# DaehwanKimLab/centrifuge

Hardware: NVIDIA H100
Metric: reads/sec (100 bp SE classification) (higher is better)
Workload: dtype u64

## Files before the change

centrifuge_b200/csrc/cf_logic.h:

```cpp
#ifndef CF_LOGIC_H_
#define CF_LOGIC_H_

#include <stdint.h>

#ifdef __CUDACC__
#define CFB_HD __host__ __device__ __forceinline__
#define CFB_HDN __host__ __device__
#else
#define CFB_HD inline
#define CFB_HDN inline
#endif

namespace cfb {

static const uint64_t kOff = 0xffffffffffffffffull;
static const uint64_t kUnk = 0xfffffffffffffffeull;
static const uint32_t kBwNone = 0xffffffffu;

struct IndexView {
	const uint64_t* sides;
	const uint64_t* ftab;
	const uint64_t* eftab;
	const uint16_t* sample16;
	const uint32_t* sample32;
// ... 245 lines not shown
	}
};

template <class T, class C> CFB_HD void ss_swap(T& a, T& b, C&) { T t = a; a = b; b = t; }

template <class T, class C> CFB_HDN void ss_unguarded_linear_insert(T* last, C comp) {
	T val = *last; T* next = last - 1;
	while(comp(val, *next)) { *last = *next; last = next; --next; }
	*last = val;
}
template <class T, class C> CFB_HDN void ss_insertion_sort(T* first, T* last, C comp) {
	if(first == last) return;
	for(T* i = first + 1; i != last; ++i) {
		if(comp(*i, *first)) { T val = *i; for(T* q = i; q != first; --q) *q = *(q - 1); *first = val; }
		else ss_unguarded_linear_insert(i, comp);
	}
}
template <class T, class C> CFB_HDN void ss_push_heap(T* first, long hole, long top, T value, C comp) {
	long parent = (hole - 1) / 2;
	while(hole > top && comp(first[parent], value)) { first[hole] = first[parent]; hole = parent; parent = (hole - 1) / 2; }
	first[hole] = value;
}
template <class T, class C> CFB_HDN void ss_adjust_heap(T* first, long hole, long len, T value, C comp) {
	const long top = hole; long child = hole;
	while(child < (len - 1) / 2) {
		child = 2 * (child + 1);
		if(comp(first[child], first[child - 1])) child--;
		first[hole] = first[child]; hole = child;
	}
	if((len & 1) == 0 && child == (len - 2) / 2) { child = 2 * (child + 1); first[hole] = first[child - 1]; hole = child - 1; }
	ss_push_heap(first, hole, top, value, comp);
}
template <class T, class C> CFB_HDN void ss_heapsort(T* first, T* last, C comp) {
	long len = (long)(last - first);
	if(len >= 2) {
		long parent = (len - 2) / 2;
		for(;;) { T v = first[parent]; ss_adjust_heap(first, parent, len, v, comp); if(parent == 0) break; parent--; }
	}
	while(last - first > 1) { --last; T v = *last; *last = *first; ss_adjust_heap(first, 0L, (long)(last - first), v, comp); }
}
template <class T, class C> CFB_HDN T* ss_partition_pivot(T* first, T* last, C comp) {
	T* mid = first + (last - first) / 2;
	T *a = first + 1, *b = mid, *c = last - 1;
	if(comp(*a, *b)) { if(comp(*b, *c)) ss_swap(*first, *b, comp); else if(comp(*a, *c)) ss_swap(*first, *c, comp); else ss_swap(*first, *a, comp); }
	else if(comp(*a, *c)) ss_swap(*first, *a, comp);
	else if(comp(*b, *c)) ss_swap(*first, *c, comp);
	else ss_swap(*first, *b, comp);
	T* lo = first + 1; T* hi = last; T* pivot = first;
	for(;;) {
		while(comp(*lo, *pivot)) ++lo;
		--hi;
		while(comp(*pivot, *hi)) --hi;
		if(!(lo < hi)) return lo;
		ss_swap(*lo, *hi, comp);
		++lo;
	}
}
template <class T, class C> CFB_HDN void std_sort(T* first, T* last, C comp) {
	const long n = (long)(last - first);
	if(n <= 0) return;
	if(n > 16) {
		int lg = 0; for(long t = n; t > 1; t >>= 1) lg++;
		T* st_first[64]; T* st_last[64]; int st_depth[64]; int sp = 0;
		st_first[0] = first; st_last[0] = last; st_depth[0] = 2 * lg; sp = 1;
		while(sp > 0) {
			--sp; T* f = st_first[sp]; T* l = st_last[sp]; int depth = st_depth[sp];
			while(l - f > 16) {
				if(depth == 0) { ss_heapsort(f, l, comp); break; }
				--depth;
				T* cut = ss_partition_pivot(f, l, comp);
				st_first[sp] = cut; st_last[sp] = l; st_depth[sp] = depth; sp++;
				l = cut;
			}
		}
		ss_insertion_sort(first, first + 16, comp);
		for(T* i = first + 16; i != last; ++i) ss_unguarded_linear_insert(i, comp);
	} else ss_insertion_sort(first, last, comp);
}

struct UnitHits {
	HitRec* L[2][2]; uint32_t n[2][2]; uint32_t rdlen[2]; int n_mates;
};

template <class F> CFB_HDN void for_each_visit(const Params& p, const UnitHits& u, F& f) {
	uint64_t maxG = p.khits;
	for(int rdi = 0; rdi < u.n_mates; rdi++) {
		int a, b;
		choose_strand(p, u.L[rdi][0], u.n[rdi][0], u.L[rdi][1], u.n[rdi][1], a, b);
		for(int fwi = a; fwi < b; fwi++) {
			const HitRec* L = u.L[rdi][fwi]; const uint32_t n = u.n[rdi][fwi];
			for(uint32_t hi = 0; hi < n; hi++) if(L[hi].len >= p.min_hitlen && hsize(L[hi]) > maxG) maxG = hsize(L[hi]);
			if(maxG > p.khits) maxG += p.khits;
			f(rdi, fwi, maxG);
		}
	}
}

struct SortAndCount {
	const Params& p; UnitHits& u; uint64_t rows;
	CFB_HD SortAndCount(const Params& p_, UnitHits& u_) : p(p_), u(u_), rows(0) {}
	CFB_HD void operator()(int rdi, int fwi, uint64_t maxG) {
		HitRec* L = u.L[rdi][fwi]; const uint32_t n = u.n[rdi][fwi];
		std_sort(L, L + n, HitLess());
		uint64_t cnt = 0;
		for(uint32_t hi = 0; hi < n; hi++) {
			if(L[hi].len <= p.min_hitlen) continue;
			if(hsize(L[hi]) == 0) continue;
			const uint64_t nelt = hsize(L[hi]) < maxG ? hsize(L[hi]) : maxG;
			if(nelt > p.ihits) continue;
			rows += nelt; cnt += nelt;
			if(cnt >= maxG) break;
		}
	}
};

struct CountRows {
	const Params& p; const UnitHits& u; uint64_t rows;
	CFB_HD CountRows(const Params& p_, const UnitHits& u_) : p(p_), u(u_), rows(0) {}
	CFB_HD void operator()(int rdi, int fwi, uint64_t maxG) {
		const HitRec* L = u.L[rdi][fwi]; const uint32_t n = u.n[rdi][fwi];
		uint64_t cnt = 0;
		for(uint32_t hi = 0; hi < n; hi++) {
			if(L[hi].len <= p.min_hitlen) continue;
			if(hsize(L[hi]) == 0) continue;
			const uint64_t nelt = hsize(L[hi]) < maxG ? hsize(L[hi]) : maxG;
			if(nelt > p.ihits) continue;
			rows += nelt; cnt += nelt;
			if(cnt >= maxG) break;
		}
	}
};

struct EmitRows {
	const Params& p; const UnitHits& u; uint64_t* out; uint64_t k; uint32_t ts, last_ts;
	CFB_HD EmitRows(const Params& p_, const UnitHits& u_, uint64_t* o) : p(p_), u(u_), out(o), k(0), ts(0), last_ts(0xffffffffu) {}
	CFB_HD void operator()(int rdi, int fwi, uint64_t maxG) {
		const HitRec* L = u.L[rdi][fwi]; const uint32_t n = u.n[rdi][fwi];
		uint64_t cnt = 0;
		for(uint32_t hi = 0; hi < n; hi++, ts++) {
			if(L[hi].len <= p.min_hitlen) continue;
			if(hsize(L[hi]) == 0) continue;
			const uint64_t nelt = hsize(L[hi]) < maxG ? hsize(L[hi]) : maxG;
			if(nelt > p.ihits) continue;
			const uint64_t head = kRowStart | ((uint64_t)(L[hi].len & 0xffffu) << 40) | ((uint64_t)(rdi & 1) << 56) | ((uint64_t)(fwi & 1) << 57)
			                    | (ts == last_ts ? kRowSameTs : 0ull);
			last_ts = ts;
			for(uint64_t e = 0; e < nelt; e++) out[k++] = ((L[hi].top + e) & kRowMask) | (e == 0 ? head : 0ull);
			cnt += nelt;
			if(cnt >= maxG) break;
		}
	}
};

struct Entry {
	uint64_t uniqueID, taxID;
	uint32_t scores[2][2], lens[2][2];
	uint32_t score, hitlen, ts;
	int32_t  pid;
	uint8_t  rank;
	uint8_t  pad[3];
};
struct TaxCnt { uint32_t count; uint32_t pad; uint64_t parent; };
struct TaxCntLess { CFB_HD bool operator()(const TaxCnt& a, const TaxCnt& b) const { return a.count < b.count || (a.count == b.count && a.parent < b.parent); } };

struct OutRec { uint64_t taxid; uint32_t score, hitlen, uid, pad; };

CFB_HD bool is_host(const IndexView& v, uint64_t taxid) {
	uint32_t lo = 0, hi = v.n_host;
	while(lo < hi) { uint32_t mid = (lo + hi) >> 1; if(v.host_taxids[mid] < taxid) lo = mid + 1; else hi = mid; }
	return lo < v.n_host && v.host_taxids[lo] == taxid;
}
CFB_HD uint32_t path_size(const Entry& e) { return e.pid < 0 ? 0u : 10u; }
CFB_HD uint64_t path_at(const IndexView& v, const Entry& e, uint32_t i) { return v.paths[(uint64_t)e.pid * 10 + i]; }

CFB_HDN uint32_t score_plan(const IndexView& v, const Params& p, const uint64_t* rows, const uint32_t* ids, uint64_t n, Entry* map) {
	uint32_t nmap = 0, ts = 0;
	for(uint64_t k = 0; k < n;) {
		const uint64_t head = rows[k];
		if(!(head & kRowSameTs)) ts++;
		const uint64_t hl = (head >> 40) & 0xffffu; const int rdi = (int)((head >> 56) & 1), fwi = (int)((head >> 57) & 1);
		uint64_t nelt = 1;
		while(k + nelt < n && !(rows[k + nelt] & kRowStart)) nelt++;
		const uint32_t* my = ids + k; k += nelt;
		const uint32_t sc = (uint32_t)((hl - 15) * (hl - 15));
		for(uint64_t e = 0; e < nelt; e++) {
			const uint32_t ref = my[e];
			bool dup = false;
			for(uint64_t q = 0; q < e; q++) if(my[q] == ref) { dup = true; break; }
			if(dup) continue;
			uint64_t taxID = ref < v.n_seqs ? v.seq_taxid[ref] : 0;
			if(v.seq_excluded && ref < v.n_seqs && v.seq_excluded[ref]) continue;
			const int32_t pid = ref < v.n_seqs ? v.seq_path[ref] : -1;
			uint8_t rank = (uint8_t)p.class_rank_slot;
			if(rank > 0 && pid >= 0) {
				for(; rank < 10; rank++) { const uint64_t t = v.paths[(uint64_t)pid * 10 + rank]; if(t != 0) { taxID = t; break; } }
			}
			uint32_t idx = 0;
			for(; idx < nmap; ++idx) {
				const bool same = rank == 0 ? ((uint64_t)ref == map[idx].uniqueID) : (taxID == map[idx].taxID);
				if(same) {
					if(map[idx].ts != ts) { map[idx].scores[rdi][fwi] += sc; map[idx].lens[rdi][fwi] += (uint32_t)hl; map[idx].ts = ts; }
					break;
				}
			}
			if(idx >= nmap) {
				Entry& n2 = map[nmap++];
				n2.uniqueID = ref; n2.taxID = taxID;
				n2.scores[0][0] = n2.scores[0][1] = n2.scores[1][0] = n2.scores[1][1] = 0;
				n2.lens[0][0] = n2.lens[0][1] = n2.lens[1][0] = n2.lens[1][1] = 0;
				n2.scores[rdi][fwi] = sc; n2.lens[rdi][fwi] = (uint32_t)hl;
				n2.score = 0; n2.hitlen = 0; n2.ts = ts; n2.pid = pid; n2.rank = rank;
			}
		}
	}
	return nmap;
}


CFB_HDN uint32_t reduce_and_emit(const IndexView& v, const Params& p, bool paired, Entry* map, uint32_t nmap,
                                 TaxCnt* tc, OutRec* out) {
	const uint32_t k = p.khits;
	for(uint32_t i = 0; i < nmap; i++) {
		Entry& h = map[i];
		const uint32_t s0 = h.scores[0][0] > h.scores[0][1] ? h.scores[0][0] : h.scores[0][1];
		const uint32_t l0 = h.lens[0][0] > h.lens[0][1] ? h.lens[0][0] : h.lens[0][1];
		if(paired) {
			const uint32_t s1 = h.scores[1][0] > h.scores[1][1] ? h.scores[1][0] : h.scores[1][1];
			const uint32_t l1 = h.lens[1][0] > h.lens[1][1] ? h.lens[1][0] : h.lens[1][1];
			h.score = s0 + s1; h.hitlen = l0 + l1;
		} else { h.score = s0; h.hitlen = l0; }
	}
	int64_t best = 0; bool only_host = false;
	for(uint32_t i = 0; i < nmap; i++) {
		if((int64_t)map[i].score > best) { best = map[i].score; only_host = is_host(v, map[i].taxID); }
		else if((int64_t)map[i].score == best) only_host |= is_host(v, map[i].taxID);
	}
	if(!only_host && nmap > k) {
		uint32_t bs = map[0].score;
		for(uint32_t i = 1; i < nmap; i++) if(bs < map[i].score) bs = map[i].score;
		for(int i = 0; i < (int)nmap; i++) {
			if(map[i].score < bs) { if(i + 1 < (int)nmap) map[i] = map[nmap - 1]; nmap--; i--; }
		}
		if(!p.tree_traverse && nmap > k) return 0;
		uint8_t rank = 0;
		while(nmap > k) {
			uint32_t ntc = 0;
			for(uint32_t i = 0; i < nmap; i++) {
				Entry& h = map[i];
				while(h.rank < rank) {
					if((uint32_t)h.rank + 1 >= path_size(h)) { h.rank = 255; break; }
					h.rank += 1; h.taxID = path_at(v, h, h.rank);
				}
				if(h.rank > rank) continue;
				const uint64_t parent = ((uint32_t)rank + 1 >= path_size(h)) ? 1 : path_at(v, h, rank + 1);
				if(parent == 0) continue;
				uint32_t j = 0;
				for(; j < ntc; j++) if(tc[j].parent == parent) { tc[j].count += 1; break; }
				if(j == ntc) { tc[ntc].count = 1; tc[ntc].pad = 0; tc[ntc].parent = parent; ntc++; }
			}
			if(ntc == 0) {
				if(rank < path_size(map[0])) { rank++; continue; } else break;
			}
			ss_heapsort(tc, tc + ntc, TaxCntLess());
			uint32_t j = ntc;
			while(j-- > 0) {
				const uint64_t parent = tc[j].parent;
				for(uint32_t i = 0; i < nmap; i++) {
					Entry& h = map[i];
					if(h.rank != rank) continue;
					const uint64_t cur_parent = ((uint32_t)rank + 1 >= path_size(h)) ? 1 : path_at(v, h, rank + 1);
					if(parent == cur_parent) { h.uniqueID = kOff; h.rank = rank + 1; h.taxID = parent; }
				}
				bool first = true;
				for(uint32_t i = 0; i < nmap; i++) {
					if(parent == map[i].taxID) {
						if(!first) { if(i + 1 < nmap) map[i] = map[nmap - 1]; nmap--; i--; }
						else first = false;
					}
				}
				if(nmap <= k) break;
			}
			++rank;
			if(rank > path_size(map[0])) break;
		}
	}
	if(!only_host && nmap > k) return 0;
	uint32_t no = 0;
	for(uint32_t i = 0; i < nmap; i++) {
		if(only_host && !is_host(v, map[i].taxID)) continue;
		OutRec r; r.taxid = map[i].taxID; r.score = map[i].score; r.hitlen = map[i].hitlen;
		r.uid = map[i].uniqueID < (uint64_t)v.n_seqs ? (uint32_t)map[i].uniqueID : 0xFFFFFFFFu; r.pad = 0;
		out[no++] = r;
	}
	return no;
}

CFB_HDN uint32_t resolve_scalar(const IndexView& v, uint64_t row, Counters* ctr) {
	const uint64_t lowmask = ((uint64_t)1 << v.off_rate) - 1;
	for(;;) {
		if(row == v.zoff) return 0;
		if((row & lowmask) == 0) {
			const uint64_t i = row >> v.off_rate;
			return v.sample32 ? v.sample32[i] : (uint32_t)v.sample16[i];
		}
		if(v.n_boundaries && row <= v.last_boundary) {
			const uint64_t b = row >> v.bshift;
			if(v.bbits[b >> 5] & (1u << (b & 31))) {
				uint32_t lo = 0, hi = v.n_boundaries;
				while(lo < hi) { uint32_t mid = (lo + hi) >> 1; if(v.brow[mid] < row) lo = mid + 1; else hi = mid; }
				if(lo < v.n_boundaries && v.brow[lo] == row) return v.sample32 ? v.bseq[lo] : (uint32_t)(uint16_t)v.bseq[lo];
			}
		}
		row = lf_scalar(v, row, bwt_char(v, row));
		if(ctr) ctr->walk_steps++;
	}
}

}
#endif
```

centrifuge_b200/csrc/cfb200.cu:

```cuda
#include "../../include/cfb200.h"
#include "cf_index.h"
#include "cf_kernels.cuh"

#include <algorithm>
#include <atomic>
#include <mutex>
#include <thread>
#include <fcntl.h>
#include <unistd.h>
#include <cstdarg>
#include <cstdio>
#include <cstring>
#include <set>
#include <string>
#include <vector>

using namespace cfb;

enum { M_DONE = 0, M_FTAB = 1, M_LF = 2, M_NEED = 3, M_FTABK = 4 };

struct Walk {
	const uint8_t* fw; uint32_t rlen; int strand; uint32_t tid;
	uint32_t cur, dep, offset, nh;
	uint64_t top, bot, fi;
// ... 796 lines not shown
	HitRec* regen; uint32_t* regen_n; unsigned long long* regen_ctr; uint64_t regen_slots; uint32_t full_cap; uint32_t keep_short;
};

__device__ uint32_t search_strand_dev(const IndexView& v, const Params& p, const uint8_t* fw, uint32_t len, int strand, HitRec* hits, uint32_t cap) {
	const ulonglong2* r16 = reinterpret_cast<const ulonglong2*>(v.rank16);
	const ulonglong2* ftab2 = reinterpret_cast<const ulonglong2*>(v.ftab2);
	const ulonglong2* ftabk = reinterpret_cast<const ulonglong2*>(v.ftabk);
	const uint32_t fc = (uint32_t)v.ftab_chars, fk = v.ftabk ? (uint32_t)v.ftabk_chars : 0u;
	auto base = [&](uint32_t d) -> int { return seq_at(fw, len, strand, len - 1 - d); };
	uint32_t cur = 0, n = 0;
	if(len == 0) return 0;
	for(;;) {
		HitRec h; h.bwoff = cur; uint32_t new_cur; bool done = false;
		const uint32_t offset = cur;
		if(len - cur < fc) { h.top = h.bot = kOff; h.len = len - offset; new_cur = len; done = true; }
		else {
			uint32_t firstn = 0xffffffffu; uint64_t fi = 0;
			const uint32_t span = (fk && len - cur >= fk) ? fk : fc;
			for(uint32_t i = 0; i < span; i++) { const int c = base(cur + i); if(c > 3) { firstn = i; break; } fi |= (uint64_t)c << (2 * i); }
			if(firstn < fc) { new_cur = cur + firstn + 1; h.top = h.bot = kOff; h.len = new_cur - offset; done = new_cur >= len; }
			else {
				uint64_t top = 0, bot = 0; uint32_t dep = 0; bool have = false;
				if(span == fk && fk > fc && firstn == 0xffffffffu) {
					const uint64_t x = __ldg(&ftabk[fi].x), width = x >> 40;
					if(width != 0 && width != kFtabkWide) { top = x & kRowMask; bot = top + width; dep = cur + fk; have = true; }
				}
				if(!have) { const ulonglong2 e = __ldg(ftab2 + (fi & ((1ull << (2 * fc)) - 1ull))); top = e.x; bot = e.y; dep = cur + fc; }
				if(bot <= top) { h.top = h.bot = kOff; h.len = dep - offset; new_cur = dep; done = dep >= len; }
				else {
					while(dep < len) {
						const int c = base(dep);
						if(c > 3) break;
						if(bot - top == 1) {
							if(v.walk8 && top < v.walk8_rows && len - dep >= 8) {
								const uint64_t e = __ldg(v.walk8 + top);
								bool ok = (e >> 56) == 8;
								for(uint32_t j = 0; ok && j < 8; j++) ok = base(dep + j) == (int)((e >> (40 + 2 * j)) & 3);
								if(ok) { top = e & kWalkRowMask; bot = top + 1; dep += 8; continue; }
							}
							const ulonglong2 e = __ldg(r16 + (top >> 6) * 4 + c);
							if(!((e.y >> (top & 63)) & 1ull)) break;
							top = v.fchr[c] + (e.x & kOccMask) + (uint64_t)__popcll(e.y & ((1ull << (top & 63)) - 1ull)); bot = top + 1; dep++;
						} else {
							const ulonglong2 et = __ldg(r16 + (top >> 6) * 4 + c);
							const ulonglong2 eb = (bot >> 6) == (top >> 6) ? et : __ldg(r16 + (bot >> 6) * 4 + c);
							const uint64_t t = v.fchr[c] + (et.x & kOccMask) + (uint64_t)__popcll(et.y & ((1ull << (top & 63)) - 1ull));
							const uint64_t b = v.fchr[c] + (eb.x & kOccMask) + (uint64_t)__popcll(eb.y & ((1ull << (bot & 63)) - 1ull));
							if(b <= t) break;
							top = t; bot = b; dep++;
						}
					}
					h.top = top; h.bot = bot; h.len = dep - offset; new_cur = dep; done = dep >= len;
				}
			}
		}
		if(n < cap) hits[n] = h;
		n++;
		cur = new_cur;
		if(done) break;
		if(h.len > p.increment) cur += 1;
		if(cur + p.min_hitlen >= len) break;
	}
	return n;
}

__device__ __forceinline__ bool load_unit(const UnitArgs& a, uint32_t unit, UnitHits& u, const uint8_t* fw[2], uint32_t found[2][2], size_t tpos[2]) {
	const uint8_t fl = a.b.flags ? a.b.flags[unit] : 3;
	u.n_mates = 0;
	for(int m = 0; m < a.b.n_mates; m++) {
		if(!((fl >> m) & 1)) continue;
		const uint32_t len = a.b.len[m][unit];
		if(len == 0) continue;
		const int r = u.n_mates++;
		const size_t t0 = ((size_t)unit * a.b.n_mates + m) * 2;
		u.rdlen[r] = len; fw[r] = a.b.bases + a.b.off[m][unit]; tpos[r] = t0;
		const uint32_t raw[2] = {a.nhits[t0], a.nhits[t0 + 1]};
		for(int st = 0; st < 2; st++) {
			if(raw[st] & kListRegen) {
				const uint32_t slot = raw[st] & 0x3fffffffu;
				u.L[r][st] = a.regen + (size_t)slot * a.full_cap; u.n[r][st] = a.regen_n[slot]; found[r][st] = 0;
			} else {
				u.L[r][st] = a.hits + (t0 + st) * a.cap; u.n[r][st] = min(nh_stored(raw[st]), a.cap); found[r][st] = nh_found(raw[st]);
			}
		}
		if(!((raw[0] | raw[1]) & kListRegen) && ((raw[0] | raw[1]) & kListNoLong)) { if(raw[0] & kListNoLong) u.n[r][0] = 0; if(raw[1] & kListNoLong) u.n[r][1] = 0; }
	}
	return u.n_mates > 0;
}

template <int MINB, bool EMIT_ONLY>
__global__ void __launch_bounds__(128, MINB) k_prep(const UnitArgs a) {
	const uint32_t unit = blockIdx.x * blockDim.x + threadIdx.x;
	const bool live = unit < a.b.n_units;
	UnitHits u; const uint8_t* fw[2]; uint32_t found[2][2]; size_t tpos[2];
	uint64_t rows = 0; bool have = false;
	if(live && (have = load_unit(a, unit, u, fw, found, tpos))) {
		if(EMIT_ONLY) { CountRows cr(a.p, u); for_each_visit(a.p, u, cr); rows = cr.rows; }
		else {
			Counters local; Counters* lc = nullptr;
			if(a.ctr) { memset(&local, 0, sizeof local); lc = &local; }
			if(!a.keep_short) for(int r = 0; r < u.n_mates; r++) {
				const bool both = u.n[r][0] > 0 && u.n[r][1] > 0;
				for(int st = 0; st < 2; st++) {
					if(u.n[r][st] == 0 || !(both || found[r][st] > 16)) continue;
					const unsigned long long slot = atomicAdd(a.regen_ctr, 1ull);
					if(slot >= a.regen_slots) { atomicExch(a.overflow, 4u); continue; }
					HitRec* L = a.regen + (size_t)slot * a.full_cap;
					const uint32_t n = search_strand_dev(a.v, a.p, fw[r], u.rdlen[r], st, L, a.full_cap);
					if(n > a.full_cap) atomicExch(a.overflow, 1u);
					u.L[r][st] = L; u.n[r][st] = min(n, a.full_cap);
					a.regen_n[slot] = u.n[r][st]; a.nhits[tpos[r] + st] = kListRegen | (uint32_t)slot;
				}
			}
			for(int r = 0; r < u.n_mates; r++) {
				const bool both = u.n[r][0] > 0 && u.n[r][1] > 0;
				for(int st = 0; st < 2; st++) {
					if(!both && u.n[r][st] <= 16) continue;
					for(uint32_t i = 0; i < u.n[r][st]; i++) {
						HitRec& h = u.L[r][st][i];
						if(h.top != kUnk) continue;
						HitRec t; uint32_t nc; bool dn;
						partial_search_scalar(a.v, fw[r], u.rdlen[r], st, h.bwoff, t, nc, dn, nullptr);
						h.top = t.top; h.bot = t.bot;
					}
				}
			}
			for(int r = 0; r < u.n_mates; r++) post_search(a.v, a.p, fw[r], u.rdlen[r], u.L[r][0], u.n[r][0], u.L[r][1], u.n[r][1], lc);
			SortAndCount sc(a.p, u);
			for_each_visit(a.p, u, sc);
			rows = sc.rows;
			if(lc) {
				atomicAdd(&a.ctr->units, 1ull);
				if(local.ext_searches) {
					atomicAdd(&a.ctr->ext_searches, local.ext_searches); atomicAdd(&a.ctr->partial_searches, local.partial_searches);
					atomicAdd(&a.ctr->ftab_probes, local.ftab_probes); atomicAdd(&a.ctr->sides_search, local.sides_search); atomicAdd(&a.ctr->lf_steps, local.lf_steps);
				}
			}
		}
		if(rows > 0xFFFFFFFFull) rows = 0xFFFFFFFFull;
	}
	const unsigned lane = threadIdx.x & 31;
	uint64_t incl = rows;
	for(int d = 1; d < 32; d <<= 1) { const uint64_t t = __shfl_up_sync(0xffffffffu, incl, d); if((int)lane >= d) incl += t; }
	const uint64_t warp_total = __shfl_sync(0xffffffffu, incl, 31);
	unsigned long long base = 0;
	if(lane == 31 && warp_total) base = atomicAdd(a.row_total, (unsigned long long)warp_total);
	base = __shfl_sync(0xffffffffu, base, 31);
	if(!live) return;
	const uint64_t off = base + incl - rows;
	a.nrows[unit] = (uint32_t)rows; a.row_off[unit] = off;
	if(rows && off + rows <= a.rows_cap) { EmitRows er(a.p, u, a.rows + off); for_each_visit(a.p, u, er); }
}

static const int kLocalMap = 4;
template <int MINB>
__global__ void __launch_bounds__(128, MINB) k_score(const UnitArgs a) {
	const uint32_t unit = blockIdx.x * blockDim.x + threadIdx.x;
	if(unit >= a.b.n_units) return;
	uint32_t no = 0;
	const uint64_t off = a.row_off[unit], n = a.nrows[unit];
	if(n > 0 && *a.row_total <= a.rows_cap) {
		const uint8_t fl = a.b.flags ? a.b.flags[unit] : 3;
		int mates = 0;
		for(int m = 0; m < a.b.n_mates; m++) if(((fl >> m) & 1) && (m ? a.b.len[1][unit] : a.b.len[0][unit]) != 0) mates++;
		Entry lmap[kLocalMap]; TaxCnt ltc[kLocalMap];
		Entry* map = n <= (uint64_t)kLocalMap ? lmap : a.entries + off;
		TaxCnt* tc = n <= (uint64_t)kLocalMap ? ltc : a.tcs + off;
		const uint32_t nmap = score_plan(a.v, a.p, a.rows + off, a.ids + off, n, map);
		no = reduce_and_emit(a.v, a.p, mates == 2, map, nmap, tc, a.recs_sparse + off);
	}
	a.nout[unit] = no;
}

static const int kScanBlock = 256, kScanPer = 4;

__global__ void __launch_bounds__(kScanBlock) k_scan_sums(const uint32_t* in, uint64_t n, uint64_t* bsum) {
	__shared__ uint64_t sh[kScanBlock];
	const uint64_t base = (uint64_t)blockIdx.x * kScanBlock * kScanPer + (uint64_t)threadIdx.x * kScanPer;
	uint64_t s = 0;
	for(int i = 0; i < kScanPer; i++) if(base + i < n) s += in[base + i];
	sh[threadIdx.x] = s; __syncthreads();
	for(int d = kScanBlock / 2; d > 0; d >>= 1) { if((int)threadIdx.x < d) sh[threadIdx.x] += sh[threadIdx.x + d]; __syncthreads(); }
	if(threadIdx.x == 0) bsum[blockIdx.x] = sh[0];
}
__global__ void k_scan_top(uint64_t* bsum, uint64_t nb, uint64_t* total) {
	__shared__ uint64_t carry;
	__shared__ uint64_t sh[1024];
	if(threadIdx.x == 0) carry = 0;
	__syncthreads();
	for(uint64_t base = 0; base < nb; base += 1024) {
		const uint64_t i = base + threadIdx.x;
		const uint64_t vv = i < nb ? bsum[i] : 0;
		sh[threadIdx.x] = vv; __syncthreads();
		for(int d = 1; d < 1024; d <<= 1) { uint64_t t = (int)threadIdx.x >= d ? sh[threadIdx.x - d] : 0; __syncthreads(); sh[threadIdx.x] += t; __syncthreads(); }
		if(i < nb) bsum[i] = carry + sh[threadIdx.x] - vv;
		__syncthreads();
		if(threadIdx.x == 1023) carry += sh[1023];
		__syncthreads();
	}
	if(threadIdx.x == 0) *total = carry;
}
__global__ void __launch_bounds__(kScanBlock) k_scan_apply(const uint32_t* in, uint64_t n, const uint64_t* bsum, const uint64_t* total, uint64_t* out) {
	__shared__ uint64_t sh[kScanBlock];
	const uint64_t base = (uint64_t)blockIdx.x * kScanBlock * kScanPer + (uint64_t)threadIdx.x * kScanPer;
	uint32_t vals[kScanPer]; uint64_t s = 0;
	for(int i = 0; i < kScanPer; i++) { vals[i] = base + i < n ? in[base + i] : 0; s += vals[i]; }
	sh[threadIdx.x] = s; __syncthreads();
	for(int d = 1; d < kScanBlock; d <<= 1) { uint64_t t = (int)threadIdx.x >= d ? sh[threadIdx.x - d] : 0; __syncthreads(); sh[threadIdx.x] += t; __syncthreads(); }
	uint64_t run = bsum[blockIdx.x] + sh[threadIdx.x] - s;
	for(int i = 0; i < kScanPer; i++) { if(base + i < n) out[base + i] = run; run += vals[i]; }
	if(blockIdx.x == 0 && threadIdx.x == 0) out[n] = *total;
}

enum { R_DONE = 0, R_WALK = 1, R_SAMPLE = 2, R_NEED = 3 };
struct ResolveArgs {
	IndexView v; const uint64_t* rows; uint32_t* ids; uint16_t* ids16; const uint64_t* total; uint64_t rows_cap;
	unsigned long long* task_ctr; uint32_t chunk; Counters* ctr;
};

template <bool COUNT>
__global__ void __launch_bounds__(kSearchThreads) k_resolve(const ResolveArgs a) {
	const unsigned lane = threadIdx.x & 31, gl = lane & 7, gbase = lane & 24, gmask = 0xFFu << gbase;
	const uint4* sides4 = reinterpret_cast<const uint4*>(a.v.sides);
	uint64_t n = *a.total; if(n > a.rows_cap) return;
	const uint64_t lowmask = ((uint64_t)1 << a.v.off_rate) - 1;
	uint64_t tnext = 0, tend = 0, idx = 0, row = 0;
	int mode = R_DONE;
	unsigned long long c_walk = 0, c_rows = 0;

	auto settle = [&](uint64_t r) -> int {
		if(r == a.v.zoff) { if(gl == 0) a.ids[idx] = 0; return R_DONE; }
		if((r & lowmask) == 0) return R_SAMPLE;
		return R_WALK;
	};
	auto next_row = [&]() -> bool {
		for(;;) {
			if(tnext >= tend) {
				unsigned long long base = 0;
				if(gl == 0) base = atomicAdd(a.task_ctr, (unsigned long long)a.chunk);
				base = __shfl_sync(gmask, base, gbase);
				if(base >= n) { mode = R_DONE; return false; }
				tnext = base; tend = base + a.chunk < n ? base + a.chunk : n;
			}
			idx = tnext++; row = a.rows[idx] & kRowMask;
			if(COUNT) c_rows++;
			mode = settle(row);
			if(mode != R_DONE) return true;
		}
	};
	next_row();
	while(__any_sync(0xffffffffu, mode != R_DONE)) {
		uint4 da = make_uint4(0, 0, 0, 0); uint32_t bits = 0, samp = 0;
		uint64_t s = 0; uint32_t off = 0; bool chk = false;
		if(mode == R_WALK) {
			s = row / 384; off = (uint32_t)(row - s * 384);
			da = __ldg(sides4 + s * 8 + gl);
			chk = a.v.n_boundaries && a.v.last_boundary > 0 && row <= a.v.last_boundary;
			if(chk) bits = __ldg(a.v.bbits + ((row >> a.v.bshift) >> 5));
		} else if(mode == R_SAMPLE) {
			if(gl == 0) samp = a.v.sample32 ? __ldg(a.v.sample32 + (row >> a.v.off_rate)) : (uint32_t)__ldg(a.v.sample16 + (row >> a.v.off_rate));
		}
		if(mode == R_SAMPLE) {
			if(gl == 0) a.ids[idx] = samp;
			next_row();
		} else if(mode == R_WALK) {
			bool found = false;
			if(chk && (bits >> ((row >> a.v.bshift) & 31)) & 1u) {
				uint32_t lo = 0, hi = a.v.n_boundaries;
				while(lo < hi) { const uint32_t mid = (lo + hi) >> 1; if(a.v.brow[mid] < row) lo = mid + 1; else hi = mid; }
				if(lo < a.v.n_boundaries && a.v.brow[lo] == row) {
					found = true;
					if(gl == 0) a.ids[idx] = a.v.sample32 ? a.v.bseq[lo] : (uint32_t)(uint16_t)a.v.bseq[lo];
				}
			}
			if(found) next_row();
			else {
				const int c = group_char(da, off, gmask, gbase);
				const uint32_t rep = (uint32_t)c * 0x55555555u;
				int nn = (int)off - 64 * (int)gl; nn = nn < 0 ? 0 : (nn > 64 ? 64 : nn);
				uint32_t cnt = gl < 6 ? lane_count(da, rep, nn) : 0u;
				cnt = group_sum(cnt, gmask);
				const uint64_t occ = group_occ(da, c, gmask, gbase);
				uint64_t r = cnt;
				if(c == 0 && s == a.v.zside && a.v.zoffc < off) r--;
				row = a.v.fchr[c] + occ + r;
				if(COUNT) c_walk++;
				mode = settle(row);
				if(mode == R_DONE) next_row();
			}
		}
	}
	if(COUNT && gl == 0 && a.ctr) { atomicAdd(&a.ctr->walk_steps, c_walk); atomicAdd(&a.ctr->rows_resolved, c_rows); }
}

template <bool COUNT>
__global__ void __launch_bounds__(kSearchThreads, 8) k_resolve_t(const ResolveArgs a) {
	const uint64_t* blocks = a.v.blocks;
	const uint64_t zblk = a.v.zoff >> 7; const uint32_t zoffb = (uint32_t)(a.v.zoff & 127);
	uint64_t n = *a.total; if(n > a.rows_cap) return;
	const uint64_t lowmask = ((uint64_t)1 << a.v.off_rate) - 1;
	uint64_t idx = 0, row = 0;
	int mode = R_NEED;
	unsigned long long c_walk = 0, c_rows = 0;
	WarpPool pool; pool.base = pool.end = 0;
	bool more = true;
	auto settle = [&](uint64_t r) -> int {
		if(r == a.v.zoff) { a.ids[idx] = 0; return R_NEED; }
		if((r & lowmask) == 0) return R_SAMPLE;
		return R_WALK;
	};
	auto next_row = [&]() { mode = R_NEED; };
	for(;;) {
		{
			const bool want = mode == R_NEED;
			if(more) {
				unsigned long long t = 0;
				const bool got = pool_take(pool, want, a.task_ctr, (unsigned long long)n, a.chunk, t);
				if(want) {
					if(got) { idx = t; row = a.rows[idx] & kRowMask; if(COUNT) c_rows++; mode = settle(row); }
					else mode = R_DONE;
				}
				if(__any_sync(0xffffffffu, want && !got)) more = false;
			} else if(want) mode = R_DONE;
		}
// ... 706 lines not shown
__global__ void __launch_bounds__(256) k_unpack(const uint64_t* __restrict__ words, const uint64_t* __restrict__ woff, uint64_t wbase, const uint32_t* __restrict__ len,
                                                uint64_t n, uint32_t W, uint8_t* bases, uint64_t* off) {
	const uint64_t t = (uint64_t)blockIdx.x * blockDim.x + threadIdx.x;
	if(t >= n * W) return;
	const uint64_t i = t / W; const uint32_t k = (uint32_t)(t - i * W);
	const uint64_t w0 = wbase + woff[i];
	if(k == 0) off[i] = w0 * 32;
	if(k * 32 >= len[i]) return;
	const uint64_t w = __ldg(words + w0 + k);
	uint32_t o[8];
	#pragma unroll
	for(int q = 0; q < 8; q++) {
		const uint32_t b = (uint32_t)(w >> (8 * q)) & 0xffu;
		o[q] = (b & 3u) | ((b & 0xcu) << 6) | ((b & 0x30u) << 12) | ((b & 0xc0u) << 18);
	}
	uint4* dst = reinterpret_cast<uint4*>(bases + (w0 + k) * 32);
	dst[0] = make_uint4(o[0], o[1], o[2], o[3]); dst[1] = make_uint4(o[4], o[5], o[6], o[7]);
}
__global__ void __launch_bounds__(256) k_set_n(const uint64_t* npos, uint64_t n, uint8_t* bases, uint64_t limit) {
	const uint64_t i = (uint64_t)blockIdx.x * blockDim.x + threadIdx.x;
	if(i < n) { const uint64_t p = npos[i]; if(p < limit) bases[p] = 4; }
}

static int stage_batch_packed(cfb_ctx* c, Slot& s, const cfb_batch_packed* b) {
	if(!b || b->n_mates < 1 || b->n_mates > 2 || !b->words || !b->len[0] || (b->n_mates == 2 && !b->len[1]) || (b->n_n && !b->n_pos))
		return fail(CFB_EINVAL, "malformed cfb_batch_packed");
	if(b->n_units >= (1ull << 30)) return fail(CFB_EINVAL, "batch too large (n_units must be < 2^30)");
	const uint64_t n = b->n_units; const int nm = b->n_mates;
	uint32_t maxlen = 0; uint64_t need_words = 0, mate_words[2] = {0, 0};
	for(int m = 0; m < nm; m++) {
		const uint32_t* L = b->len[m]; uint32_t mx = 0; uint64_t w = 0;
		for(uint64_t i = 0; i < n; i++) { const uint32_t l = L[i]; mx = l > mx ? l : mx; w += (l + 31u) >> 5; }
		maxlen = std::max(maxlen, mx); mate_words[m] = w; need_words += w;
	}
	if(need_words != b->n_words) return fail(CFB_EINVAL, "cfb_batch_packed: n_words is %llu, the lengths need %llu", (unsigned long long)b->n_words, (unsigned long long)need_words);
	if(maxlen > 60000) return fail(CFB_EINVAL, "read longer than 60000 bases");
	const uint64_t scan_blocks = (n + kScanBlock * kScanPer - 1) / (kScanBlock * kScanPer);
	CK(s.d_bases.ensure(b->n_words * 32 + 64)); CK(s.d_off.ensure(n * nm + 1)); CK(s.d_len.ensure(n * nm)); CK(s.d_flags.ensure(n));
	CK(s.d_words.ensure(b->n_words + 1)); CK(s.d_npos.ensure(b->n_n + 1)); CK(s.d_wlen.ensure(n + 1)); CK(s.d_woff.ensure(n + 2)); CK(s.bsum.ensure(scan_blocks + 1));
	auto pinned = [](const void* p) -> bool {
		cudaPointerAttributes at;
		if(cudaPointerGetAttributes(&at, p) != cudaSuccess) { cudaGetLastError(); return false; }
		return at.type == cudaMemoryTypeHost;
	};
	const uint64_t* src_words = b->words;
	if(!pinned(b->words)) { CK(s.h_words.ensure(b->n_words)); memcpy(s.h_words.p, b->words, b->n_words * 8); src_words = s.h_words.p; }
	CK(cudaMemcpyAsync(s.d_words.p, src_words, b->n_words * 8, cudaMemcpyHostToDevice, s.st));
	CK(s.h_len.ensure(n * nm)); CK(s.h_flags.ensure(n));
	for(int m = 0; m < nm; m++) {
		const uint32_t* sl = b->len[m];
		if(!pinned(sl)) { memcpy(s.h_len.p + m * n, sl, n * 4); sl = s.h_len.p + m * n; }
		CK(cudaMemcpyAsync(s.d_len.p + m * n, sl, n * 4, cudaMemcpyHostToDevice, s.st));
	}
	if(b->n_n) {
		const uint64_t* sp = b->n_pos;
		if(!pinned(sp)) { CK(s.h_off.ensure(b->n_n)); memcpy(s.h_off.p, sp, b->n_n * 8); sp = s.h_off.p; }
		CK(cudaMemcpyAsync(s.d_npos.p, sp, b->n_n * 8, cudaMemcpyHostToDevice, s.st));
	}
	if(b->flags && pinned(b->flags)) CK(cudaMemcpyAsync(s.d_flags.p, b->flags, n, cudaMemcpyHostToDevice, s.st));
	else { if(b->flags) memcpy(s.h_flags.p, b->flags, n); else memset(s.h_flags.p, 3, n); CK(cudaMemcpyAsync(s.d_flags.p, s.h_flags.p, n, cudaMemcpyHostToDevice, s.st)); }
	const uint32_t W = (maxlen + 31) / 32;
	uint64_t wbase = 0;
	CK(cudaMemsetAsync(s.scal.p + 5, 0, 8, s.st));
	for(int m = 0; m < nm && n; m++) {
		k_wlen<<<(unsigned)((n + 255) / 256), 256, 0, s.st>>>(s.d_len.p + m * n, n, s.d_wlen.p);
		k_scan_sums<<<(unsigned)scan_blocks, kScanBlock, 0, s.st>>>(s.d_wlen.p, n, s.bsum.p);
		k_scan_top<<<1, 1024, 0, s.st>>>(s.bsum.p, scan_blocks, (uint64_t*)(s.scal.p + 5));
		k_scan_apply<<<(unsigned)scan_blocks, kScanBlock, 0, s.st>>>(s.d_wlen.p, n, s.bsum.p, (const uint64_t*)(s.scal.p + 5), s.d_woff.p);
		if(W) k_unpack<<<(unsigned)((n * W + 255) / 256), 256, 0, s.st>>>(s.d_words.p, s.d_woff.p, wbase, s.d_len.p + m * n, n, W, s.d_bases.p, s.d_off.p + m * n);
		c->launches += 5;
		wbase += mate_words[m];
	}
	if(b->n_n) { k_set_n<<<(unsigned)((b->n_n + 255) / 256), 256, 0, s.st>>>(s.d_npos.p, b->n_n, s.d_bases.p, b->n_words * 32); c->launches++; }
	CK(cudaGetLastError());
	s.bv.bases = s.d_bases.p; s.bv.flags = s.d_flags.p; s.bv.n_units = (uint32_t)n; s.bv.n_mates = nm;
	for(int m = 0; m < 2; m++) { s.bv.off[m] = m < nm ? s.d_off.p + m * n : nullptr; s.bv.len[m] = m < nm ? s.d_len.p + m * n : nullptr; }
	s.n_units = n; s.n_bases = b->n_words * 32; s.maxlen = maxlen;
	return CFB_OK;
}

static int enqueue_kernels(cfb_ctx* c, Slot& s, int stage, bool time_it) {
	const uint64_t n = s.n_units; const int nm = s.bv.n_mates;
	const uint64_t ntasks = n * nm * 2;
	const uint32_t ublocks = (uint32_t)((n + 127) / 128);
	const uint64_t scan_blocks = (n + kScanBlock * kScanPer - 1) / (kScanBlock * kScanPer);
	if(n == 0) return CFB_OK;
	int variant = c->group;
	if(variant == 1) { if(s.maxlen > 320) variant = 16; else if(s.maxlen > 160) variant = 100; else if(s.maxlen > 128) variant = 101; }
	const bool pooled = variant == 1 || variant == 100 || variant == 101;
	const bool keep_short = !pooled || c->prm.min_hitlen < kLongLen || c->keep_short;
	if(stage == 0) {
		if(s.cap == 0) {
			s.full_cap = s.maxlen / 4 + 8;
			s.cap = keep_short ? s.full_cap : s.maxlen / kLongLen + 2;
		}
		CK(s.hits.ensure(ntasks * s.cap)); CK(s.nhits.ensure(ntasks));
		if(!keep_short) {
			s.regen_slots = std::max<uint64_t>(s.regen_slots, c->regen_slots0 ? c->regen_slots0 : std::max<uint64_t>(ntasks / 32, 1024));
			CK(s.regen.ensure(s.regen_slots * s.full_cap)); CK(s.regen_n.ensure(s.regen_slots));
			CK(cudaMemsetAsync(s.scal.p + 6, 0, sizeof(unsigned long long), s.st));
		}
		const uint32_t W = (s.maxlen + 31) / 32 + 1;
		CK(s.pk.ensure(ntasks * W + 2)); CK(s.nm.ensure(ntasks * W + 2)); CK(s.nrows.ensure(n)); CK(s.row_off.ensure(n + 1));
		CK(s.bsum.ensure(scan_blocks + 1)); CK(s.nout.ensure(n)); CK(s.out_off.ensure(n + 1)); CK(s.rec_off32.ensure(n + 1));
		s.rows_cap = std::max<uint64_t>(s.rows_cap, c->rows_cap0 ? c->rows_cap0 : std::max<uint64_t>(n * 12, 4096));
	}
	CK(s.rows.ensure(s.rows_cap)); CK(s.ids.ensure(s.rows_cap)); CK(s.entries.ensure(s.rows_cap)); CK(s.tcs.ensure(s.rows_cap)); CK(s.sparse.ensure(s.rows_cap));
	s.dense_cap = s.rows_cap; CK(s.dense.ensure(s.dense_cap));
	CK(cudaMemsetAsync(s.scal.p, 0, 4 * sizeof(unsigned long long), s.st));
	if(time_it) CK(cudaEventRecord(s.ev[0], s.st));
	Counters* ctr = c->count ? c->d_ctr : nullptr;
	if(c->count && stage == 0) CK(cudaMemsetAsync(c->d_ctr, 0, sizeof(Counters), s.st));
	UnitArgs ua; ua.v = c->view; ua.p = c->prm; ua.b = s.bv; ua.hits = s.hits.p; ua.nhits = s.nhits.p; ua.cap = s.cap;
	ua.nrows = s.nrows.p; ua.row_off = s.row_off.p; ua.row_total = s.scal.p + 3; ua.rows = s.rows.p; ua.ids = s.ids.p; ua.rows_cap = s.rows_cap;
	ua.entries = s.entries.p; ua.tcs = s.tcs.p; ua.recs_sparse = s.sparse.p; ua.nout = s.nout.p;
	ua.overflow = (unsigned int*)(s.scal.p + 2); ua.ctr = ctr;
	ua.regen = s.regen.p; ua.regen_n = s.regen_n.p; ua.regen_ctr = s.scal.p + 6; ua.regen_slots = s.regen_slots; ua.full_cap = s.full_cap; ua.keep_short = keep_short ? 1u : 0u;
	if(stage == 0) {
		SearchArgs sa; sa.v = c->view; sa.p = c->prm; sa.b = s.bv; sa.hits = s.hits.p; sa.nhits = s.nhits.p; sa.cap = s.cap;
		const uint32_t W = (s.maxlen + 31) / 32 + 1;
		sa.pk = s.pk.p; sa.nm = s.nm.p; sa.W = W; sa.jump_w = c->jump_w; sa.keep_short = keep_short ? 1u : 0u;
		{ PackArgs pa; pa.b = s.bv; pa.pk = s.pk.p; pa.nm = s.nm.p; pa.W = W;
		  k_pack<<<(unsigned)((ntasks * W + 127) / 128), 128, 0, s.st>>>(pa); c->launches++; }
		sa.task_ctr = (unsigned int*)(s.scal.p + 0); sa.task_ctr64 = s.scal.p + 0; sa.ntasks = (uint32_t)ntasks; sa.overflow = (unsigned int*)(s.scal.p + 2); sa.ctr = ctr;
		const int lanes = (variant == 16 || pooled) ? 1 : variant;
		int occ = 1;
		CK(cudaOccupancyMaxActiveBlocksPerMultiprocessor(&occ, search_kernel(variant, c->count), kSearchThreads, 0));
		const uint64_t resident = (uint64_t)c->ix->sm_count * (uint64_t)std::max(occ, 1);
		const uint64_t per_block = kSearchThreads / lanes;
		const uint64_t groups = resident * per_block;
		uint64_t chunk = ntasks / (groups * 8); sa.chunk = (uint32_t)std::min<uint64_t>(std::max<uint64_t>(chunk, 1), 16);
		if(pooled) {
			const uint64_t warps = resident * (kSearchThreads / 32);
			sa.chunk = (uint32_t)std::min<uint64_t>(std::max<uint64_t>(ntasks / (warps * 4), 32), 256);
		}
		const int blocks = (int)std::min<uint64_t>(resident, (ntasks + per_block - 1) / per_block);
		search_kernel(variant, c->count)<<<blocks, kSearchThreads, 0, s.st>>>(sa);
		c->launches++;
		if(time_it) CK(cudaEventRecord(s.ev[1], s.st));
		k_prep<8, false><<<ublocks, 128, 0, s.st>>>(ua); c->launches++;
	} else {
		if(time_it) CK(cudaEventRecord(s.ev[1], s.st));
		k_prep<8, true><<<ublocks, 128, 0, s.st>>>(ua); c->launches++;
	}
	if(time_it) CK(cudaEventRecord(s.ev[2], s.st));
	ResolveArgs ra; ra.v = c->view; ra.rows = s.rows.p; ra.ids = s.ids.p; ra.ids16 = nullptr; ra.total = (const uint64_t*)(s.scal.p + 3); ra.rows_cap = s.rows_cap;
	ra.task_ctr = s.scal.p + 1; ra.chunk = c->resolve_mode >= 2 ? 64 : (c->resolve_mode == 1 ? 128 : 4); ra.ctr = ctr;
	if(c->resolve_mode == 3 && c->count != 1) k_lookup<<<c->ix->sm_count * 8, 256, 0, s.st>>>(ra);
	else if(c->resolve_mode >= 2) { if(c->count) k_resolve_c<true, false><<<c->resolve_blocks, kSearchThreads, 0, s.st>>>(ra); else k_resolve_c<false, false><<<c->resolve_blocks, kSearchThreads, 0, s.st>>>(ra); }
	else if(c->resolve_mode == 1) { if(c->count) k_resolve_t<true><<<c->resolve_blocks, kSearchThreads, 0, s.st>>>(ra); else k_resolve_t<false><<<c->resolve_blocks, kSearchThreads, 0, s.st>>>(ra); }
	else { if(c->count) k_resolve<true><<<c->resolve_blocks, kSearchThreads, 0, s.st>>>(ra); else k_resolve<false><<<c->resolve_blocks, kSearchThreads, 0, s.st>>>(ra); }
	c->launches++;
	if(time_it) CK(cudaEventRecord(s.ev[3], s.st));
	k_score<12><<<ublocks, 128, 0, s.st>>>(ua); c->launches++;
	k_scan_sums<<<(unsigned)scan_blocks, kScanBlock, 0, s.st>>>(s.nout.p, n, s.bsum.p);
	k_scan_top<<<1, 1024, 0, s.st>>>(s.bsum.p, scan_blocks, (uint64_t*)(s.scal.p + 4));
	k_scan_apply<<<(unsigned)scan_blocks, kScanBlock, 0, s.st>>>(s.nout.p, n, s.bsum.p, (const uint64_t*)(s.scal.p + 4), s.out_off.p);
	k_compact<<<(unsigned)((n + 1 + 127) / 128), 128, 0, s.st>>>((uint32_t)n, s.row_off.p, s.out_off.p, s.sparse.p, s.dense.p, s.rec_off32.p, s.dense_cap, (unsigned int*)(s.scal.p + 2));
	c->launches += 4;
	s.folded = false;
	if(c->fold_records && !s.is_text) {
		const uint32_t nsp = c->cnt.n;
		CK(s.cnt.ensure(3ull * nsp)); CK(cudaMemsetAsync(s.cnt.p, 0, 3ull * nsp * 8, s.st));
		FoldArgs fa; fa.sp_taxid = c->cnt.d_taxid.p; fa.n_sp = nsp; fa.rec_off = s.rec_off32.p; fa.recs = s.dense.p; fa.n_units = (uint32_t)n; fa.n_mates = nm;
		fa.khits = c->prm.khits; fa.len[0] = s.bv.len[0]; fa.len[1] = s.bv.len[1]; fa.flags = s.bv.flags; fa.sp = s.cnt.p;
		k_fold_counts<<<ublocks, 128, 0, s.st>>>(fa); c->launches++;
		s.folded = true;
	}
	if(time_it) CK(cudaEventRecord(s.ev[4], s.st));
	s.d2h_recs = 0;
	if(s.want_host) {
		const uint64_t guess = std::min<uint64_t>(s.dense_cap, (uint64_t)((double)n * c->rec_ratio * 1.05) + 4096);
		CK(s.h_recs.ensure(guess + 1)); CK(s.h_rec_off.ensure(n + 1));
		CK(cudaMemcpyAsync(s.h_rec_off.p, s.rec_off32.p, (n + 1) * 4, cudaMemcpyDeviceToHost, s.st));
		CK(cudaMemcpyAsync(s.h_recs.p, s.dense.p, guess * sizeof(OutRec), cudaMemcpyDeviceToHost, s.st));
		s.d2h_recs = guess;
	}
	CK(cudaMemcpyAsync(s.h_scal.p, s.scal.p, 8 * sizeof(unsigned long long), cudaMemcpyDeviceToHost, s.st));
	CK(cudaGetLastError());
	return CFB_OK;
}

static int finish_batch(cfb_ctx* c, Slot& s, bool time_it, bool to_host, cfb_result* out) {
	if(s.n_units == 0) { if(out) { out->n_units = 0; out->n_recs = 0; out->rec_off = nullptr; out->recs = nullptr; } return CFB_OK; }
	for(int attempt = 0; attempt < 8; attempt++) {
		CK(cudaStreamSynchronize(s.st));
		const unsigned ovf = (unsigned)(s.h_scal.p[2] & 0xffffffffu);
		const uint64_t total_rows = s.h_scal.p[3];
		if(ovf == 4) {
			s.regen_slots = s.h_scal.p[6] + s.h_scal.p[6] / 4 + 1024; s.reran = true;
			int rc = enqueue_kernels(c, s, 0, time_it); if(rc) return rc;
			continue;
		}
		if(ovf == 1) {
			s.cap = s.maxlen + 2; s.full_cap = s.maxlen + 2; s.reran = true;
			int rc = enqueue_kernels(c, s, 0, time_it); if(rc) return rc;
			continue;
		}
		if(total_rows > s.rows_cap) {
			s.rows_cap = total_rows + total_rows / 4 + 1024; s.reran = true;
			int rc = enqueue_kernels(c, s, 1, time_it); if(rc) return rc;
			continue;
		}
		if(ovf != 0) return fail(CFB_ECUDA, "internal capacity error %u", ovf);
		break;
	}
	const uint64_t nrec = s.h_scal.p[4];
	c->regen_lists += s.h_scal.p[6]; c->regen_tasks += (uint64_t)s.n_units * (uint64_t)s.bv.n_mates * 2;
	if(s.folded) {
		const uint32_t n3 = 3 * c->cnt.n;
		k_cnt_commit<<<(n3 + 255) / 256, 256, 0, s.st>>>(s.cnt.p, c->cnt.total.p, n3); c->launches++;
		CK(cudaEventRecord(s.ev[5], s.st)); s.commit_pending = true;
		s.folded = false; c->cnt.reduced = false;
	}
	if(to_host) {
		if(s.n_units) c->rec_ratio = std::max(c->rec_ratio * 0.98, (double)nrec / (double)s.n_units);
		if(!s.want_host || nrec > s.d2h_recs) {
			const uint64_t have = s.want_host ? s.d2h_recs : 0;
			if(nrec + 1 > s.h_recs.cap) {
				CK(s.h_recs.ensure(nrec + 1));
				if(nrec) CK(cudaMemcpyAsync(s.h_recs.p, s.dense.p, nrec * sizeof(OutRec), cudaMemcpyDeviceToHost, s.st));
			} else if(nrec > have) CK(cudaMemcpyAsync(s.h_recs.p + have, s.dense.p + have, (nrec - have) * sizeof(OutRec), cudaMemcpyDeviceToHost, s.st));
			if(!s.want_host) { CK(s.h_rec_off.ensure(s.n_units + 1)); CK(cudaMemcpyAsync(s.h_rec_off.p, s.rec_off32.p, (s.n_units + 1) * 4, cudaMemcpyDeviceToHost, s.st)); }
			CK(cudaStreamSynchronize(s.st));
		}
	}
	if(out) { out->n_units = s.n_units; out->n_recs = nrec; out->rec_off = s.h_rec_off.p; out->recs = reinterpret_cast<const cfb_rec*>(s.h_recs.p); }
	return CFB_OK;
}

extern "C" int cfb_classify_submit(cfb_ctx* c, int slot, const cfb_batch* b) {
	if(!c || slot < 0 || slot >= kSlots - 1) return fail(CFB_EINVAL, "bad ctx/slot");
	CK(cudaSetDevice(c->ix->device));
	Slot& s = c->slots[slot];
	if(s.pending) return fail(CFB_EINVAL, "slot %d still has an un-waited batch", slot);
	int rc = stage_batch(c, s, b); if(rc) return rc;
	s.cap = 0; s.want_host = true; s.is_text = false;
	rc = enqueue_kernels(c, s, 0, false); if(rc) return rc;
	s.pending = true;
	return CFB_OK;
}
extern "C" int cfb_classify_submit_packed(cfb_ctx* c, int slot, const cfb_batch_packed* b) {
	if(!c || slot < 0 || slot >= kSlots - 1) return fail(CFB_EINVAL, "bad ctx/slot");
	CK(cudaSetDevice(c->ix->device));
	Slot& s = c->slots[slot];
	if(s.pending) return fail(CFB_EINVAL, "slot %d still has an un-waited batch", slot);
	int rc = stage_batch_packed(c, s, b); if(rc) return rc;
	s.cap = 0; s.want_host = true; s.is_text = false;
	rc = enqueue_kernels(c, s, 0, false); if(rc) return rc;
	s.pending = true;
	return CFB_OK;
}
extern "C" int cfb_pack_batch(const cfb_batch* in, uint64_t* words, uint64_t words_cap, uint64_t* n_pos, uint64_t npos_cap, uint64_t* n_words, uint64_t* n_n) {
	if(!in || !n_words || !n_n || in->n_mates < 1 || in->n_mates > 2) return fail(CFB_EINVAL, "cfb_pack_batch: bad argument");
	uint64_t w = 0, nn = 0; bool fits = true;
	for(int m = 0; m < in->n_mates; m++) for(uint64_t i = 0; i < in->n_units; i++) {
		const uint8_t* p = in->bases + in->off[m][i]; const uint32_t len = in->len[m][i];
		for(uint32_t k = 0; k < len; k += 32) {
			uint64_t v = 0; const uint32_t cnt = std::min<uint32_t>(32, len - k);
			for(uint32_t j = 0; j < cnt; j++) {
				const uint8_t c = p[k + j];
				if(c > 3) { if(n_pos && nn < npos_cap) n_pos[nn] = (w << 5) | j; else fits = false; nn++; }
				else v |= (uint64_t)c << (2 * j);
			}
			if(words && w < words_cap) words[w] = v; else fits = false;
			w++;
		}
	}
	*n_words = w; *n_n = nn;
	return fits ? CFB_OK : fail(CFB_EINVAL, "cfb_pack_batch: buffers too small (%llu words, %llu N positions needed)", (unsigned long long)w, (unsigned long long)nn);
}
extern "C" int cfb_classify_wait(cfb_ctx* c, int slot, cfb_result* out) {
	if(!c || slot < 0 || slot >= kSlots - 1 || !out) return fail(CFB_EINVAL, "bad ctx/slot");
	CK(cudaSetDevice(c->ix->device));
	Slot& s = c->slots[slot];
	if(!s.pending) return fail(CFB_EINVAL, "slot %d has no submitted batch", slot);
	s.pending = false;
	return finish_batch(c, s, false, true, out);
}
extern "C" int cfb_classify_batch(cfb_ctx* c, const cfb_batch* b, cfb_result* out) {
	int rc = cfb_classify_submit(c, 0, b); if(rc) return rc;
	return cfb_classify_wait(c, 0, out);
}

extern "C" int cfb_batch_upload(cfb_ctx* c, const cfb_batch* b, cfb_dbatch** out) {
	if(!c || !out) return fail(CFB_EINVAL, "null argument");
	if(c->resident_used) return fail(CFB_EINVAL, "only one resident batch per ctx");
	CK(cudaSetDevice(c->ix->device));
	Slot& s = c->slots[kSlots - 1];
	int rc = stage_batch(c, s, b); if(rc) return rc;
	CK(cudaStreamSynchronize(s.st));
	s.cap = 0; s.is_text = false;
	c->resident.slot = kSlots - 1; c->resident.n_units = s.n_units; c->resident_used = true;
	*out = &c->resident;
	return CFB_OK;
}
extern "C" void cfb_dbatch_free(cfb_ctx* c, cfb_dbatch*) { if(c) c->resident_used = false; }
extern "C" int cfb_classify_resident(cfb_ctx* c, cfb_dbatch* d, float* ms, uint64_t* n_recs) {
	return cfb_classify_resident_range(c, d, 0, d ? d->n_units : 0, ms, n_recs);
}
extern "C" int cfb_classify_resident_range(cfb_ctx* c, cfb_dbatch* d, uint64_t first, uint64_t count, float* ms, uint64_t* n_recs) {
	if(!c || !d) return fail(CFB_EINVAL, "null argument");
	if(first + count > d->n_units) return fail(CFB_EINVAL, "cfb_classify_resident_range: units [%llu, %llu) exceed the uploaded batch", (unsigned long long)first, (unsigned long long)(first + count));
	CK(cudaSetDevice(c->ix->device));
	Slot& s = c->slots[d->slot];
	const uint64_t N = d->n_units; const int nmates = s.bv.n_mates;
	s.bv.flags = s.d_flags.p + first; s.bv.n_units = (uint32_t)count; s.n_units = count;
// ... 65 lines not shown
```

Baseline: 261.9 million.

## Stage score rows, maps and records in shared memory per warp

The scoring kernel now has each warp claim a contiguous slice of a per-block shared-memory pool. It copies its units' rows and ids into that slice, builds the Entry map, tax counts and output records there, and then writes the records back to global memory cooperatively and coalesced. This replaces the small per-thread local arrays and the scattered global scratch used for larger units. Entry.uniqueID shrinks to 32 bits to cut shared-memory footprint. Warps whose span does not fit in the pool fall back to global buffers, and the larger static shared allocation may reduce occupancy below the MINB=12 target.

Result: faster. 274.4 million (median of 6 runs) (+4.8%).

```diff
diff --git a/centrifuge_b200/csrc/cf_logic.h b/centrifuge_b200/csrc/cf_logic.h
--- a/centrifuge_b200/csrc/cf_logic.h
+++ b/centrifuge_b200/csrc/cf_logic.h
@@ -421,8 +421,10 @@
 	}
 };
 
+static const uint32_t kUidOff = 0xffffffffu;
 struct Entry {
-	uint64_t uniqueID, taxID;
+	uint64_t taxID;
+	uint32_t uniqueID;
 	uint32_t scores[2][2], lens[2][2];
 	uint32_t score, hitlen, ts;
 	int32_t  pid;
@@ -466,7 +468,7 @@
 			}
 			uint32_t idx = 0;
 			for(; idx < nmap; ++idx) {
-				const bool same = rank == 0 ? ((uint64_t)ref == map[idx].uniqueID) : (taxID == map[idx].taxID);
+				const bool same = rank == 0 ? (ref == map[idx].uniqueID) : (taxID == map[idx].taxID);
 				if(same) {
 					if(map[idx].ts != ts) { map[idx].scores[rdi][fwi] += sc; map[idx].lens[rdi][fwi] += (uint32_t)hl; map[idx].ts = ts; }
 					break;
@@ -538,7 +540,7 @@
 					Entry& h = map[i];
 					if(h.rank != rank) continue;
 					const uint64_t cur_parent = ((uint32_t)rank + 1 >= path_size(h)) ? 1 : path_at(v, h, rank + 1);
-					if(parent == cur_parent) { h.uniqueID = kOff; h.rank = rank + 1; h.taxID = parent; }
+					if(parent == cur_parent) { h.uniqueID = kUidOff; h.rank = rank + 1; h.taxID = parent; }
 				}
 				bool first = true;
 				for(uint32_t i = 0; i < nmap; i++) {
@@ -558,7 +560,7 @@
 	for(uint32_t i = 0; i < nmap; i++) {
 		if(only_host && !is_host(v, map[i].taxID)) continue;
 		OutRec r; r.taxid = map[i].taxID; r.score = map[i].score; r.hitlen = map[i].hitlen;
-		r.uid = map[i].uniqueID < (uint64_t)v.n_seqs ? (uint32_t)map[i].uniqueID : 0xFFFFFFFFu; r.pad = 0;
+		r.uid = map[i].uniqueID < v.n_seqs ? map[i].uniqueID : 0xFFFFFFFFu; r.pad = 0;
 		out[no++] = r;
 	}
 	return no;
diff --git a/centrifuge_b200/csrc/cfb200.cu b/centrifuge_b200/csrc/cfb200.cu
--- a/centrifuge_b200/csrc/cfb200.cu
+++ b/centrifuge_b200/csrc/cfb200.cu
@@ -972,24 +972,64 @@
 	if(rows && off + rows <= a.rows_cap) { EmitRows er(a.p, u, a.rows + off); for_each_visit(a.p, u, er); }
 }
 
-static const int kLocalMap = 4;
+static const int kScoreThreads = 128;
+static const uint32_t kScorePool = 128;
+static const uint32_t kNoSlot = 0xffffffffu;
 template <int MINB>
-__global__ void __launch_bounds__(128, MINB) k_score(const UnitArgs a) {
+__global__ void __launch_bounds__(kScoreThreads, MINB) k_score(const UnitArgs a) {
+	__shared__ uint64_t s_rows[kScorePool]; __shared__ uint32_t s_ids[kScorePool];
+	__shared__ Entry s_map[kScorePool]; __shared__ TaxCnt s_tc[kScorePool]; __shared__ OutRec s_recs[kScorePool];
+	__shared__ uint32_t s_used;
+	if(threadIdx.x == 0) s_used = 0;
+	__syncthreads();
 	const uint32_t unit = blockIdx.x * blockDim.x + threadIdx.x;
-	if(unit >= a.b.n_units) return;
+	const unsigned lane = threadIdx.x & 31;
+	const bool valid = unit < a.b.n_units;
+	const bool fits = *a.row_total <= a.rows_cap;
+	const uint64_t n = valid && fits ? a.nrows[unit] : 0, off = valid && fits ? a.row_off[unit] : 0;
+	const uint64_t base = __shfl_sync(0xffffffffu, off, 0);
+	uint64_t span = n ? off + n - base : 0;
+	for(int d = 16; d > 0; d >>= 1) span = max(span, __shfl_xor_sync(0xffffffffu, span, d));
+	uint32_t slot = kNoSlot;
+	if(lane == 0 && span) {
+		uint32_t cur = *(volatile uint32_t*)&s_used;
+		while(span <= kScorePool - cur) {
+			const uint32_t old = atomicCAS(&s_used, cur, cur + (uint32_t)span);
+			if(old == cur) { slot = cur; break; }
+			cur = old;
+		}
+	}
+	slot = __shfl_sync(0xffffffffu, slot, 0);
+	const bool sh = slot != kNoSlot;
+	if(sh) {
+		for(uint32_t j = lane; j < (uint32_t)span; j += 32) { s_rows[slot + j] = a.rows[base + j]; s_ids[slot + j] = a.ids[base + j]; }
+		__syncwarp();
+	}
+	const uint32_t loc = sh ? slot + (uint32_t)(off - base) : 0u;
 	uint32_t no = 0;
-	const uint64_t off = a.row_off[unit], n = a.nrows[unit];
-	if(n > 0 && *a.row_total <= a.rows_cap) {
+	if(n > 0) {
 		const uint8_t fl = a.b.flags ? a.b.flags[unit] : 3;
 		int mates = 0;
 		for(int m = 0; m < a.b.n_mates; m++) if(((fl >> m) & 1) && (m ? a.b.len[1][unit] : a.b.len[0][unit]) != 0) mates++;
-		Entry lmap[kLocalMap]; TaxCnt ltc[kLocalMap];
-		Entry* map = n <= (uint64_t)kLocalMap ? lmap : a.entries + off;
-		TaxCnt* tc = n <= (uint64_t)kLocalMap ? ltc : a.tcs + off;
-		const uint32_t nmap = score_plan(a.v, a.p, a.rows + off, a.ids + off, n, map);
-		no = reduce_and_emit(a.v, a.p, mates == 2, map, nmap, tc, a.recs_sparse + off);
-	}
-	a.nout[unit] = no;
+		const uint64_t* rows = sh ? s_rows + loc : a.rows + off;
+		const uint32_t* ids = sh ? s_ids + loc : a.ids + off;
+		Entry* map = sh ? s_map + loc : a.entries + off;
+		TaxCnt* tc = sh ? s_tc + loc : a.tcs + off;
+		OutRec* out = sh ? s_recs + loc : a.recs_sparse + off;
+		const uint32_t nmap = score_plan(a.v, a.p, rows, ids, n, map);
+		no = reduce_and_emit(a.v, a.p, mates == 2, map, nmap, tc, out);
+	}
+	if(valid) a.nout[unit] = no;
+	if(sh) {
+		__syncwarp();
+		for(int u = 0; u < 32; u++) {
+			const uint32_t cnt = __shfl_sync(0xffffffffu, no, u) * 3u, l = __shfl_sync(0xffffffffu, loc, u);
+			const uint64_t o = __shfl_sync(0xffffffffu, off, u);
+			const uint64_t* src = reinterpret_cast<const uint64_t*>(s_recs + l);
+			uint64_t* dst = reinterpret_cast<uint64_t*>(a.recs_sparse + o);
+			for(uint32_t w = lane; w < cnt; w += 32) dst[w] = src[w];
+		}
+	}
 }
 
 static const int kScanBlock = 256, kScanPer = 4;
@@ -2002,7 +2042,7 @@
 	else { if(c->count) k_resolve<true><<<c->resolve_blocks, kSearchThreads, 0, s.st>>>(ra); else k_resolve<false><<<c->resolve_blocks, kSearchThreads, 0, s.st>>>(ra); }
 	c->launches++;
 	if(time_it) CK(cudaEventRecord(s.ev[3], s.st));
-	k_score<12><<<ublocks, 128, 0, s.st>>>(ua); c->launches++;
+	k_score<12><<<ublocks, kScoreThreads, 0, s.st>>>(ua); c->launches++;
 	k_scan_sums<<<(unsigned)scan_blocks, kScanBlock, 0, s.st>>>(s.nout.p, n, s.bsum.p);
 	k_scan_top<<<1, 1024, 0, s.st>>>(s.bsum.p, scan_blocks, (uint64_t*)(s.scal.p + 4));
 	k_scan_apply<<<(unsigned)scan_blocks, kScanBlock, 0, s.st>>>(s.nout.p, n, s.bsum.p, (const uint64_t*)(s.scal.p + 4), s.out_off.p);
```
